# therealadityashankar/hey-buddy

Measured on AMD Instinct MI355X. Metric: audio clips/sec featurized+trained, 1.5 s @16 kHz, 1/2/4/8 GPU, higher is better.
Workload: dtype f32

## Files before the change

### hey-buddy_amd/csrc/hbk_augment_plan.h

```cpp
#pragma once

#include <algorithm>
#include <cmath>
#include <cstdarg>
#include <cstdint>
#include <cstdio>
#include <numeric>
#include <string>
#include <vector>

namespace hbk {
namespace {

constexpr int kPlanOk = 0, kPlanErrArg = -1, kPlanErrUnsupported = -3;

inline std::string strf(const char* fmt, ...) {
  char buf[512];
  va_list ap;
  va_start(ap, fmt);
  vsnprintf(buf, sizeof(buf), fmt, ap);
  va_end(ap);
  return buf;
}

// ... 79 lines not shown
    return kPlanErrUnsupported;
  }
  return kPlanOk;
}

struct PitchLayout {
  int64_t y = 0;
  int64_t taps = 0;
  int64_t yr = 0;
  int64_t sp = 0;
  int64_t key = 0;
  int64_t ord = 0;
  int64_t gord = 0;
  int64_t total = 0;
};

inline PitchLayout pitch_layout(const PitchGeometry& a, int64_t n) {
  PitchLayout w;
  w.y = 0;
  w.taps = up256(n * a.l1 * 4);
  w.yr = w.taps + up256(int64_t(kPsPhaseMax) * kPsTapMax * 4);
  w.sp = w.yr + up256(n * 8);
  w.key = w.sp + up256(n * 8);
  w.ord = w.key + up256(n * 8);
  w.gord = w.ord + up256(n * 4);
  w.total = w.gord + up256(n * 4);
  return w;
}

struct PitchKnobs {
  bool span = true;
  bool pair = true;
  bool resample_valu = false;
};

struct Grid {
  unsigned x = 1, y = 1, block = 0;
};

struct PitchLaunches {
  bool pair = false;
  int groups = 0;
  Grid taps, span, rank_clips, group, rank_groups, vocoder, resample;
  bool resample_mfma = true;
};

inline PitchLaunches pitch_launches(const PitchGeometry& a, int64_t n, const PitchKnobs& k) {
  PitchLaunches p;
  p.pair = k.span && k.pair;
  p.groups = static_cast<int>((n + kPvClips - 1) / kPvClips);
  p.taps = Grid{unsigned((a.nw * kPsTapMax + 255) / 256), 1, 256};
  p.span = Grid{unsigned((n + 3) / 4), 1, 256};
  p.rank_clips = Grid{unsigned((n + 63) / 64), 1, 1024};
  p.group = Grid{unsigned((p.groups + 255) / 256), 1, 256};
  p.rank_groups = Grid{unsigned((p.groups + 63) / 64), 1, 1024};
  p.vocoder = Grid{unsigned(p.groups), 1, unsigned(128 * kPvClips)};
  const int res_frames = (a.L + a.nw - 1) / a.nw;
  p.resample_mfma = !(k.resample_valu || a.nw > 128);
  p.resample = p.resample_mfma ? Grid{unsigned((res_frames + kRsFrames - 1) / kRsFrames), unsigned(n), 256}
                               : Grid{unsigned((res_frames + kPsResFrames - 1) / kPsResFrames), unsigned(n), 128};
  return p;
}

struct BandStopLayout {
  int64_t sums = 0;
  int64_t taps = 0;
// ... 74 lines not shown
```

### hey-buddy_amd/csrc/hbk_pitch.hip

```cpp
#include <atomic>
#include <cstdlib>

#include "hbk_augment_plan.h"
#include "hbk_common.h"

namespace hbk {
namespace {

static_assert(kPsTapMax == HBK_PITCH_SHIFT_MAX_TAPS, "the resampler's tap rows");
static_assert(kPlanOk == HBK_OK && kPlanErrArg == HBK_ERR_ARG && kPlanErrUnsupported == HBK_ERR_UNSUPPORTED,
              "the planner's status values");
#ifndef HBK_PV_ABLATE
#define HBK_PV_ABLATE 0
#endif
#ifndef HBK_PV_F32STATE
#define HBK_PV_F32STATE 0
#endif
#ifndef HBK_PV_RESTART
#if HBK_PV_F32STATE
#define HBK_PV_RESTART 128
#else
#define HBK_PV_RESTART 1024
#endif
#endif
constexpr int kPvRestart = HBK_PV_RESTART;
#if HBK_PV_F32STATE
typedef float pv_t;
#else
typedef double pv_t;
#endif

struct PitchArgs {
  const float* x;
  int64_t x_stride;
// ... 679 lines not shown
  }
  float tp[kPsTapMax];
  const float* tr = a.taps + min(ph, a.nw - 1) * kPsTapMax;
#pragma unroll
  for (int q = 0; q < kPsTapMax; ++q) tp[q] = tr[q];
  __syncthreads();
  if (ph >= a.nw) return;
  float* out = a.out + static_cast<int64_t>(a.idx[e]) * a.out_stride;
  for (int p = 0; p < kPairs; ++p) {
    const int i = (f0 + 2 * p) * a.nw + ph, i1 = i + a.nw;
    if (i >= a.L) break;
    cf v = {0.f, 0.f};
    if (i < a.target) {
      const float4* w = reinterpret_cast<const float4*>(ys2[p]);
#pragma unroll
      for (int q2 = 0; q2 < kPsTapMax / 2; ++q2) {
        const float4 ww = w[q2];
        v = __builtin_elementwise_fma(cf{tp[2 * q2], tp[2 * q2]}, cf{ww.x, ww.y}, v);
        v = __builtin_elementwise_fma(cf{tp[2 * q2 + 1], tp[2 * q2 + 1]}, cf{ww.z, ww.w}, v);
      }
    }
    out[i] = v.x;
    if (i1 < a.L) out[i1] = i1 < a.target ? v.y : 0.f;
  }
}


typedef _Float16 rs_h8 __attribute__((ext_vector_type(8)));
typedef float rs_f4 __attribute__((ext_vector_type(4)));
__device__ __forceinline__ void rs_split(float v, _Float16& h, _Float16& l) {
  h = static_cast<_Float16>(v);
  l = static_cast<_Float16>(v - static_cast<float>(h));
}
__global__ void __launch_bounds__(256) ps_resample_mfma_kernel(PitchArgs a) {
  __shared__ __attribute__((aligned(16))) _Float16 wh[kRsFrames][kRsLd];
  __shared__ __attribute__((aligned(16))) _Float16 wl[kRsFrames][kRsLd];
  __shared__ float red[4];
  const int tid = threadIdx.x, lane = tid & 63, wave = tid >> 6;
  const int e = blockIdx.y, f0 = blockIdx.x * kRsFrames;
  const float* y = a.y + static_cast<int64_t>(e) * a.l1;
  const int2 yr = a.yr[e];
  if (ps_window_silent(a, yr, e, f0 * a.orig - a.width, f0, kRsFrames, tid, 256)) return;
  constexpr int kPairs = kRsFrames * kRsK / 2, kPer = kPairs / 256;
  float v0[kPer], v1[kPer];
  float mx = 0.f;
#pragma unroll
  for (int u = 0; u < kPer; ++u) {
    const int p = tid + 256 * u, fr = p / (kRsK / 2), q = 2 * (p - fr * (kRsK / 2));
    const int src = (f0 + fr) * a.orig - a.width + q;
    const int s0 = min(max(src, 0), a.l1 - 1), s1 = min(max(src + 1, 0), a.l1 - 1);
    const float x0 = y[s0], x1 = y[s1];
    v0[u] = (src >= yr.x && src < yr.y && q < kPsTapMax) ? x0 : 0.f;
    v1[u] = (src + 1 >= yr.x && src + 1 < yr.y && q + 1 < kPsTapMax) ? x1 : 0.f;
    mx = fmaxf(mx, fmaxf(fabsf(v0[u]), fabsf(v1[u])));
  }
  const int n = lane & 15, kq = lane >> 4;
  rs_h8 bh[2][5], bl[2][5];
#pragma unroll
  for (int t = 0; t < 2; ++t) {
    const int ph = min(16 * (2 * wave + t) + n, a.nw - 1);
    const float* tr = a.taps + ph * kPsTapMax;
#pragma unroll
    for (int ks = 0; ks < 5; ++ks)
#pragma unroll
      for (int j = 0; j < 8; ++j) {
        const int q = 32 * ks + 8 * kq + j;
        const float tv = tr[min(q, kPsTapMax - 1)];
        _Float16 h, l;
        rs_split(q < kPsTapMax ? tv * 1024.f : 0.f, h, l);
        bh[t][ks][j] = h;
        bl[t][ks][j] = l;
      }
  }
  for (int o = 32; o >= 1; o >>= 1) mx = fmaxf(mx, __shfl_xor(mx, o, 64));
  if (lane == 0) red[wave] = mx;
  __syncthreads();
  mx = fmaxf(fmaxf(red[0], red[1]), fmaxf(red[2], red[3]));
  const int ex = mx > 0.f ? min(14 - ilogbf(mx), 100) : 0;
  const float scale = ldexpf(1.f, ex), unscale = ldexpf(1.f, -ex - 10);
#pragma unroll
  for (int u = 0; u < kPer; ++u) {
    const int p = tid + 256 * u, fr = p / (kRsK / 2), q = 2 * (p - fr * (kRsK / 2));
    _Float16 h0, l0, h1, l1;
    rs_split(v0[u] * scale, h0, l0);
    rs_split(v1[u] * scale, h1, l1);
    wh[fr][q] = h0;
    wh[fr][q + 1] = h1;
    wl[fr][q] = l0;
    wl[fr][q + 1] = l1;
  }
  __syncthreads();
  float* out = a.out + static_cast<int64_t>(a.idx[e]) * a.out_stride;
#pragma unroll
  for (int ft = 0; ft < kRsFrames / 16; ++ft) {
    rs_f4 acc[2] = {{0.f, 0.f, 0.f, 0.f}, {0.f, 0.f, 0.f, 0.f}};
#pragma unroll
    for (int ks = 0; ks < 5; ++ks) {
      const rs_h8 ah = *reinterpret_cast<const rs_h8*>(&wh[16 * ft + n][32 * ks + 8 * kq]);
      const rs_h8 al = *reinterpret_cast<const rs_h8*>(&wl[16 * ft + n][32 * ks + 8 * kq]);
#pragma unroll
      for (int t = 0; t < 2; ++t) {
        acc[t] = __builtin_amdgcn_mfma_f32_16x16x32_f16(ah, bh[t][ks], acc[t], 0, 0, 0);
        acc[t] = __builtin_amdgcn_mfma_f32_16x16x32_f16(ah, bl[t][ks], acc[t], 0, 0, 0);
        acc[t] = __builtin_amdgcn_mfma_f32_16x16x32_f16(al, bh[t][ks], acc[t], 0, 0, 0);
      }
    }
#pragma unroll
    for (int t = 0; t < 2; ++t) {
      const int ph = 16 * (2 * wave + t) + n;
#pragma unroll
      for (int j = 0; j < 4; ++j) {
        const int i = (f0 + 16 * ft + 4 * kq + j) * a.nw + ph;
        if (ph < a.nw && i < a.L) out[i] = i < a.target ? acc[t][j] * unscale : 0.f;
      }
    }
  }
}

PitchKnobs read_pitch_knobs() {
  PitchKnobs k;
  const char* s = getenv("HBK_PS_SPAN");
  k.span = !(s && s[0] == '0');
  s = getenv("HBK_PS_PAIR");
  k.pair = !(s && s[0] == '0');
  k.resample_valu = getenv("HBK_PS_RESAMPLE_VALU") != nullptr;
  return k;
}

int vocoder_lds_opt_in() {
  constexpr int kDevices = 64;
  static std::atomic<bool> done[kDevices];
  int dev = -1;
  HBK_HIP(hipGetDevice(&dev));
  const bool tracked = dev >= 0 && dev < kDevices;
  if (tracked && done[dev].load(std::memory_order_acquire)) return HBK_OK;
  HBK_HIP(hipFuncSetAttribute(reinterpret_cast<const void*>(ps_vocoder_kernel),
                              hipFuncAttributeMaxDynamicSharedMemorySize, int(sizeof(PvShared))));
  if (tracked) done[dev].store(true, std::memory_order_release);
  return HBK_OK;
}

template <typename... Params, typename... Args>
void launch(void (*kernel)(Params...), const Grid& g, size_t lds, hipStream_t st, Args... args) {
  hipLaunchKernelGGL(kernel, dim3(g.x, g.y), dim3(g.block), lds, st, args...);
}

}

#ifdef HBK_PHASE_TIMING
int pv_phase_take(unsigned long long* out) {
  if (hipMemcpyFromSymbol(out, HIP_SYMBOL(g_pv_phase), sizeof(unsigned long long) * 5) != hipSuccess) return -2;
  unsigned long long z[5] = {};
  (void)hipMemcpyToSymbol(HIP_SYMBOL(g_pv_phase), z, sizeof(z));
  return 0;
}
#endif

}

extern "C" {

int64_t hbk_pitch_shift_workspace_size(int64_t n, int64_t T, int32_t sample_rate, int32_t num, int32_t den) {
  hbk::PitchGeometry g;
  std::string err;
  if (n <= 0 || hbk::pitch_geometry(T, sample_rate, num, den, g, err) != HBK_OK) return 0;
  return hbk::pitch_layout(g, n).total;
}

int hbk_pitch_shift(const float* x, int64_t x_stride, int64_t n, const int32_t* idx, int64_t T, int32_t sample_rate,
                    int32_t num, int32_t den, float* out, int64_t out_stride, void* workspace,
                    int64_t workspace_bytes, void* stream) {
  using namespace hbk;
  if (n < 0) return arg_error("negative n");
  if (n == 0) return HBK_OK;
  if (n > 65535) return arg_error("n > 65535 per call");
  if (!x || !idx || !out || !workspace) return arg_error("NULL pointer");
  PitchGeometry g;
// ... 2 lines not shown
  if (rc != HBK_OK) {
    set_error("%s", err.c_str());
    return rc;
  }
  if (x_stride < T || out_stride < T) return arg_error("stride < T");
  const PitchLayout off = pitch_layout(g, n);
  if (workspace_bytes < off.total) return arg_error("workspace too small (hbk_pitch_shift_workspace_size)");
  const PitchKnobs knobs = read_pitch_knobs();
  const PitchLaunches L = pitch_launches(g, n, knobs);
  unsigned char* w = static_cast<unsigned char*>(workspace);
  PitchArgs a{};
  a.x = x;
  a.x_stride = x_stride;
  a.idx = idx;
  a.n = static_cast<int>(n);
  a.out = out;
  a.out_stride = out_stride;
  a.L = g.L, a.f_in = g.f_in, a.f_out = g.f_out, a.l1 = g.l1;
  a.orig = g.orig, a.nw = g.nw, a.width = g.width, a.target = g.target;
  a.rate = g.rate;
  a.y = reinterpret_cast<float*>(w + off.y);
  a.taps = reinterpret_cast<float*>(w + off.taps);
  a.yr = reinterpret_cast<int2*>(w + off.yr);
  a.span = knobs.span ? 1 : 0;
  if (L.pair) {
    a.sp = reinterpret_cast<int2*>(w + off.sp);
    a.key = reinterpret_cast<uint64_t*>(w + off.key);
    a.ord = reinterpret_cast<int32_t*>(w + off.ord);
    a.gord = reinterpret_cast<int32_t*>(w + off.gord);
  }
  const int lds_rc = vocoder_lds_opt_in();
  if (lds_rc != HBK_OK) return lds_rc;
  hipStream_t st = as_stream(stream);
  launch(ps_taps_kernel, L.taps, 0, st, a);
  HBK_LAUNCH_CHECK("ps_taps_kernel");
  if (L.pair) {
    launch(ps_span_kernel, L.span, 0, st, a);
    HBK_LAUNCH_CHECK("ps_span_kernel");
    launch(ps_rank_kernel, L.rank_clips, 0, st, static_cast<const uint64_t*>(a.key), a.n, a.ord);
    HBK_LAUNCH_CHECK("ps_rank_kernel");
    launch(ps_group_kernel, L.group, 0, st, a, L.groups);
    HBK_LAUNCH_CHECK("ps_group_kernel");
    launch(ps_rank_kernel, L.rank_groups, 0, st, static_cast<const uint64_t*>(a.key), L.groups, a.gord);
    HBK_LAUNCH_CHECK("ps_rank_kernel");
  }
  launch(ps_vocoder_kernel, L.vocoder, sizeof(PvShared), st, a);
  HBK_LAUNCH_CHECK("ps_vocoder_kernel");
  launch(L.resample_mfma ? ps_resample_mfma_kernel : ps_resample_kernel, L.resample, 0, st, a);
  HBK_LAUNCH_CHECK(L.resample_mfma ? "ps_resample_mfma_kernel" : "ps_resample_kernel");
  return HBK_OK;
}

}
```

### hey-buddy_amd/heybuddy/_native.py

```python
from __future__ import annotations

import ctypes
import os
import threading
from typing import Optional

import torch

__all__ = ["HBKError", "HBKUnavailable", "lib", "check", "stream_ptr", "require_device",
           "LIB_PATH"]

LIB_PATH = os.environ.get(
    "HBK_LIB",
    os.path.join(os.path.dirname(os.path.dirname(os.path.abspath(__file__))), "lib", "libhbk.so"),
)


class HBKError(RuntimeError):
    """A libhbk.so entry point returned a non-zero status."""


class HBKUnavailable(HBKError):
    """libhbk.so (or a HIP device) is not available: the HIP path cannot run."""


_lock = threading.Lock()
_lib: Optional[ctypes.CDLL] = None

_c_int64 = ctypes.c_int64
_c_int = ctypes.c_int
_c_float = ctypes.c_float
_vp = ctypes.c_void_p

_PROTOS = {
# ... 19 lines not shown
                                     ctypes.POINTER(ctypes.c_double),
                                     ctypes.POINTER(ctypes.c_double),
                                     ctypes.POINTER(ctypes.c_int32)]),
    "hbk_embed_workspace_size": (_c_int, [_vp, _c_int64, ctypes.POINTER(_c_int64)]),
    "hbk_embed_clips": (_c_int, [_vp, _vp, _c_int64, _c_int64, _vp, _vp, _c_int64, _vp]),
    "hbk_embed_split_info": (_c_int, [_vp, ctypes.c_int32, ctypes.POINTER(_c_int64)]),
    "hbk_embed_clips_front": (_c_int, [_vp, _vp, _c_int64, _c_int64, ctypes.c_int32, _vp, _vp, _c_int64, _vp]),
    "hbk_embed_clips_back": (_c_int, [_vp, _vp, _c_int64, ctypes.c_int32, _vp, _vp, _c_int64, _vp]),
    "hbk_embed_windows": (_c_int, [_vp, _vp, _c_int64, _vp, _vp, _c_int64, _vp]),
    "hbk_nan_rows_workspace_size": (_c_int64, [_c_int64]),
    "hbk_nan_rows_fix": (_c_int, [_vp, _c_int64, _c_int64, ctypes.c_uint64, _vp, _c_int64, _vp]),
    "hbk_embed_range_status": (_c_int, [_vp, ctypes.POINTER(ctypes.c_int32), ctypes.c_int32, _vp]),
    "hbk_reverb_plan_create": (_c_int, [_c_int64, ctypes.POINTER(_vp)]),
    "hbk_reverb_plan_destroy": (_c_int, [_vp]),
    "hbk_reverb_spectrum": (_c_int, [_vp, _vp, _c_int64, _c_int64, _vp, _vp]),
    "hbk_augment": (_c_int, [_vp, _vp, _c_int64, _c_int64, _vp, _c_int64, _vp, _vp, _vp, _vp, _vp,
                             _vp, _c_int64, _vp]),
    "hbk_colored_noise": (_c_int, [_vp, _vp, _c_int64, _c_int64, _vp, _c_int64, ctypes.c_uint64, _c_int64, _vp,
                                   _vp, _c_float, _vp, _c_int64, _vp, _c_int64, _vp]),
    "hbk_augment_colored": (_c_int, [_vp, _vp, _c_int64, _c_int64, _vp, _c_int64, _vp, _vp, _vp, _vp, _vp,
                                     _vp, _c_int64, ctypes.c_uint64, _c_int64, _vp, _vp, _c_float, _vp, _c_int64,
                                     _vp, _c_int64, _vp, _c_int64, _vp]),
    "hbk_colored_noise_workspace_size": (_c_int64, [_c_int64, _c_int64]),
    "hbk_colored_noise_ws": (_c_int, [_vp, _vp, _c_int64, _c_int64, _vp, _c_int64, ctypes.c_uint64, _c_int64, _vp,
                                      _vp, _c_float, _vp, _c_int64, _vp, _c_int64, _vp, _c_int64, _vp]),
    "hbk_tanh_distortion": (_c_int, [_vp, _c_int64, _c_int64, _vp, _vp, _c_int64, _vp, _c_int64, _vp]),
    "hbk_band_stop_workspace_size": (_c_int64, [_c_int64, ctypes.c_int32, ctypes.c_int32, _vp]),
    "hbk_band_stop": (_c_int, [_vp, _vp, _c_int64, _c_int64, _vp, _vp, ctypes.c_int32, _vp, _vp, _vp, _vp,
                               ctypes.c_int32, _vp, _vp, _vp, _c_int64, _vp, _c_int64, _vp]),
    "hbk_pitch_shift_workspace_size": (_c_int64, [_c_int64, _c_int64, ctypes.c_int32, ctypes.c_int32,
                                                  ctypes.c_int32]),
    "hbk_pitch_shift": (_c_int, [_vp, _c_int64, _c_int64, _vp, _c_int64, ctypes.c_int32, ctypes.c_int32,
                                 ctypes.c_int32, _vp, _c_int64, _vp, _c_int64, _vp]),
    "hbk_seven_band_eq": (_c_int, [_vp, _c_int64, _c_int64, _vp, _vp, _c_int64, _vp, _c_int64, _vp]),
    "hbk_place_clips": (_c_int, [_vp, _c_int64, _c_int64, _vp, _vp, _vp, _c_int64, _c_int64, _vp]),
    "hbk_place_clips_idx": (_c_int, [_vp, _c_int64, _c_int64, _vp, _vp, _vp, _c_int64, _vp, _c_int64, _c_int64,
                                     _vp]),
    "hbk_seven_band_eq_src": (_c_int, [_vp, _c_int64, _c_int64, _vp, _vp, _c_int64, _vp, _c_int64,
                                       _vp, _c_int64, _vp, _vp, _vp]),
    "hbk_tanh_distortion_src": (_c_int, [_vp, _c_int64, _c_int64, _vp, _vp, _c_int64, _vp, _c_int64,
                                         _vp, _c_int64, _vp, _vp, _vp]),
    "hbk_reverb_plan_set_source": (_c_int, [_vp, _vp, _c_int64, _vp, _vp]),
    "hbk_mlp_set_step_scalars": (_c_int, [_vp, _vp]),
    "hbk_mlp_plan_create": (_c_int, [ctypes.c_int32] * 4 + [ctypes.POINTER(_vp)]),
    "hbk_mlp_plan_create_ex": (_c_int, [ctypes.c_int32] * 6 + [ctypes.POINTER(_vp)]),
    "hbk_mlp_act_forward": (_c_int, [_vp, _c_int64, ctypes.c_int32, ctypes.c_int32, ctypes.c_int32, _vp, _vp]),
    "hbk_mlp_act_backward": (_c_int, [_vp, _vp, _c_int64, ctypes.c_int32, ctypes.c_int32, ctypes.c_int32, _vp,
                                      _vp]),
    "hbk_mlp_plan_create_half": (_c_int, [ctypes.c_int32] * 6 + [_vp, ctypes.POINTER(_vp)]),
    "hbk_mlp_half_layout": (_c_int, [_vp, _vp, ctypes.c_int32]),
    "hbk_mlp_plan_destroy": (_c_int, [_vp]),
    "hbk_mlp_layout": (_c_int, [_vp, ctypes.POINTER(_c_int64), _vp, ctypes.c_int32]),
    "hbk_mlp_workspace_size": (_c_int, [_vp, _c_int64, ctypes.POINTER(_c_int64)]),
    "hbk_mlp_forward": (_c_int, [_vp, _vp, _vp, _c_int64, _vp, _vp, _c_float, ctypes.c_uint64,
                                 _vp, _c_int64, _vp]),
    "hbk_mlp_train_fwd_bwd": (_c_int, [_vp, _vp, _vp, _vp, _c_int64, _c_float, _c_float, _c_float,
                                       _c_float, ctypes.c_uint64, _vp, _vp, _vp, _c_int64, _vp]),
    "hbk_mlp_gate_adam": (_c_int, [_vp, _vp, _vp, _vp, _vp, _vp, _vp, _vp, ctypes.c_int32,
                                   _c_float, _c_float, _c_float, _c_float, _vp]),
    "hbk_mlp_fused_supported": (_c_int, [_vp, ctypes.POINTER(ctypes.c_int32)]),
    "hbk_mlp_step_variant": (_c_int, [_vp, _c_int64, _vp, ctypes.POINTER(ctypes.c_int32)]),
    "hbk_mlp_step_plan_info": (_c_int, [_vp, _c_int64, _vp, ctypes.POINTER(ctypes.c_int32), ctypes.c_int32]),
    "hbk_mlp_step_fwd_bwd": (_c_int, [_vp, _vp, _vp, _c_int64, _vp, _c_int64, _vp, _c_int64, _vp, _c_int64,
                                      _c_int64, _vp, ctypes.c_int32, _vp, _c_int64, _c_float, _c_float,
                                      _c_float, _c_float, ctypes.c_uint64, _vp, _vp, _c_int64, ctypes.c_int32,
                                      _vp, _c_int64, _vp]),
# ... 14 lines not shown


class GraphOp(ctypes.Structure):
    _fields_ = [
        ("kind", ctypes.c_int32), ("kh", ctypes.c_int32), ("kw", ctypes.c_int32),
        ("cin", ctypes.c_int32), ("cout", ctypes.c_int32), ("act", ctypes.c_int32),
        ("alpha", ctypes.c_float), ("weight", _vp), ("bias", _vp),
    ]


def exported_symbols() -> list[str]:
    return list(_PROTOS)


def lib() -> ctypes.CDLL:
    global _lib
    if _lib is not None:
        return _lib
    with _lock:
        if _lib is not None:
            return _lib
        if not os.path.exists(LIB_PATH):
            raise HBKUnavailable(
                f"libhbk.so not found at {LIB_PATH}; build it with "
                "`python hey-buddy_amd/build.py` (the HIP path has no fallback)")
        try:
            handle = ctypes.CDLL(LIB_PATH, mode=ctypes.RTLD_GLOBAL)
        except OSError as e:
            raise HBKUnavailable(f"cannot load {LIB_PATH}: {e}") from e
        for name, (res, args) in _PROTOS.items():
            fn = getattr(handle, name)
            fn.restype = res
            fn.argtypes = args
        _lib = handle
        return _lib


def check(rc: int, what: str = "") -> None:
    if rc != 0:
        msg = lib().hbk_last_error().decode(errors="replace")
        raise HBKError(f"{what}: status {rc}: {msg}")


def require_device(device: Optional[torch.device | int] = None) -> torch.device:
    lib()
    if not torch.cuda.is_available():
        raise HBKUnavailable("no HIP device visible: the hey-buddy MI355X path needs a GPU")
    if device is None:
        return torch.device("cuda", torch.cuda.current_device())
    if isinstance(device, int):
        return torch.device("cuda", device)
    device = torch.device(device)
    if device.type != "cuda":
        raise HBKUnavailable(f"device {device} is not a HIP device")
    return device if device.index is not None else torch.device("cuda", torch.cuda.current_device())


def stream_ptr(device: Optional[torch.device] = None) -> int:
    return torch.cuda.current_stream(device).cuda_stream


def ptr(t: torch.Tensor) -> int:
    return t.data_ptr()
```

### include/hbk.h

```cpp
#ifndef HBK_H
#define HBK_H

#include <stdint.h>

#ifdef __cplusplus
extern "C" {
#endif

typedef enum {
  HBK_OK = 0,
  HBK_ERR_ARG = -1,
  HBK_ERR_HIP = -2,
  HBK_ERR_UNSUPPORTED = -3
} hbk_status;

const char* hbk_version(void);
const char* hbk_last_error(void);
int hbk_device_count(int* count);
int hbk_stream_create_cu_mask(const uint32_t* cu_mask, int n_words, void** stream);
int hbk_stream_destroy(void* stream);

int hbk_profile_mark(int32_t tag, void* stream);

typedef struct hbk_mel_plan hbk_mel_plan;
// ... 157 lines not shown
                const float* noise_ring, int64_t ring_len, const int64_t* noise_off,
                const float* snr_db, const float* spectra, const int32_t* spec_idx,
                const float* gain, float* out, int64_t out_stride, void* stream);

int hbk_colored_noise(const hbk_reverb_plan* plan, const float* x, int64_t n_clips, int64_t x_stride,
                      const float* white, int64_t white_stride, uint64_t seed, int64_t clips_per_noise,
                      const float* f_decay, const float* snr_db, float sample_rate, const int32_t* idx,
                      int64_t n_entries, float* out, int64_t out_stride, void* stream);
int64_t hbk_colored_noise_workspace_size(int64_t n_clips, int64_t clips_per_noise);
int hbk_colored_noise_ws(const hbk_reverb_plan* plan, const float* x, int64_t n_clips, int64_t x_stride,
                         const float* white, int64_t white_stride, uint64_t seed, int64_t clips_per_noise,
                         const float* f_decay, const float* snr_db, float sample_rate, const int32_t* idx,
                         int64_t n_entries, float* out, int64_t out_stride, void* workspace, int64_t workspace_bytes,
                         void* stream);

int hbk_augment_colored(const hbk_reverb_plan* plan, const float* x, int64_t n_clips, int64_t x_stride,
                        const float* noise_ring, int64_t ring_len, const int64_t* noise_off,
                        const float* snr_db, const float* spectra, const int32_t* spec_idx,
                        const float* gain, const float* white, int64_t white_stride, uint64_t seed,
                        int64_t clips_per_noise, const float* c_f_decay, const float* c_snr_db,
                        float sample_rate, const int32_t* c_idx, int64_t c_n_entries, float* out,
                        int64_t out_stride, void* workspace, int64_t workspace_bytes, void* stream);

#define HBK_BAND_STOP_CIRCULAR_MAX_HALF 512
#define HBK_BAND_STOP_PARTITION_TAPS 11521
int64_t hbk_band_stop_workspace_size(int64_t n, int32_t n_filters, int32_t n_spectra, void* stream);
int hbk_band_stop(const hbk_reverb_plan* plan, const float* x, int64_t x_stride, int64_t n, const int32_t* idx,
                  const int32_t* filt, int32_t n_filters, const float* f_lo, const float* f_hi,
                  const int32_t* f_half, const int32_t* f_spec0, int32_t n_spectra, const int32_t* s_filt,
                  const int32_t* s_part, float* out, int64_t out_stride, void* workspace, int64_t workspace_bytes,
                  void* stream);

#define HBK_PITCH_SHIFT_MAX_TAPS 144
int64_t hbk_pitch_shift_workspace_size(int64_t n, int64_t T, int32_t sample_rate, int32_t num, int32_t den);
int hbk_pitch_shift(const float* x, int64_t x_stride, int64_t n, const int32_t* idx, int64_t T, int32_t sample_rate,
                    int32_t num, int32_t den, float* out, int64_t out_stride, void* workspace,
                    int64_t workspace_bytes, void* stream);

int hbk_seven_band_eq(const float* x, int64_t n_clips, int64_t x_stride, const double* coef, const int32_t* idx,
                      int64_t n_entries, float* out, int64_t out_stride, void* stream);

int hbk_tanh_distortion(const float* x, int64_t n_clips, int64_t x_stride, const float* amount,
                        const int32_t* idx, int64_t n_entries, float* out, int64_t out_stride, void* stream);

int hbk_place_clips(const float* src, int64_t n_clips, int64_t src_stride, const int32_t* src_len,
                    const int32_t* pre, float* out, int64_t out_stride, int64_t T, void* stream);
int hbk_place_clips_idx(const float* src, int64_t n_clips, int64_t src_stride, const int32_t* src_len,
                        const int32_t* pre, const int32_t* idx, int64_t n_entries, float* out,
                        int64_t out_stride, int64_t T, void* stream);

int hbk_seven_band_eq_src(const float* x, int64_t n_clips, int64_t x_stride, const double* coef,
                          const int32_t* idx, int64_t n_entries, float* out, int64_t out_stride,
                          const float* src, int64_t src_stride, const int32_t* src_len,
                          const int32_t* src_pre, void* stream);
int hbk_tanh_distortion_src(const float* x, int64_t n_clips, int64_t x_stride, const float* amount,
                            const int32_t* idx, int64_t n_entries, float* out, int64_t out_stride,
                            const float* src, int64_t src_stride, const int32_t* src_len,
                            const int32_t* src_pre, void* stream);
int hbk_reverb_plan_set_source(hbk_reverb_plan* plan, const float* src, int64_t src_stride,
                               const int32_t* src_len, const int32_t* src_pre);

#ifdef __cplusplus
}
#endif

#endif
// ... 1 lines not shown
```

### hey-buddy_amd/csrc/hbk_clip_ops.hip

```cpp
#include <algorithm>

#include "hbk_aug_dev.h"

namespace hbk {
namespace {

struct TanhArgs {
  const float* x;
  int64_t x_stride;
  float* out;
  int64_t out_stride;
  int64_t n_clips;
  const float* amount;
  const int32_t* idx;
  int64_t n_entries;
  SrcView view;
};

__device__ __forceinline__ unsigned abs_bits(float v, int s) {
  return s < kT ? (__builtin_bit_cast(unsigned, v) & 0x7FFFFFFFu) : 0xFFFFFFFFu;
}

__global__ void __launch_bounds__(kThreads) __attribute__((amdgpu_waves_per_eu(8)))
tanh_distortion_kernel(TanhArgs a) {
  __shared__ unsigned hist[4096];
  __shared__ float red[32];
  __shared__ unsigned pick[2];
  constexpr int kPer = (kT + kThreads - 1) / kThreads;
  const int64_t n_iter = a.idx ? a.n_entries : a.n_clips;
  for (int64_t e = blockIdx.x; e < n_iter; e += gridDim.x) {
    const int64_t clip = a.idx ? a.idx[e] : e;
    const int tid = opaque_tid();
    const float* x = a.x + clip * a.x_stride;
    float* out = a.out + clip * a.out_stride;
    const float amt = a.amount[clip];
    if (amt != amt) {
      if (out != x) copy_clip(x, out, tid);
      continue;
    }
    float xr[kPer];
    const int pre = a.view.pre ? a.view.pre[clip] : -1, len = a.view.pre ? a.view.len[clip] : 0;
    if (pre >= 0) {
      const int n = min(len, kT);
      const float* row = n > 0 ? a.view.src + clip * a.view.stride : x;
      const int t = opaque_tid();
      const int w0 = __builtin_amdgcn_readfirstlane(t & ~63);
#pragma unroll
      for (int u = 0; u < kPer; ++u) xr[u] = load_placed_wave(row, pre, n, w0 + u * kThreads, t & 63);
    } else {
    const int t = opaque_tid();
#pragma unroll
    for (int u = 0; u < kPer; ++u) {
      const int s = t + u * kThreads;
      xr[u] = s < kT ? *reinterpret_cast<const float*>(reinterpret_cast<const char*>(x) + (static_cast<uint32_t>(s) << 2))
                     : 0.f;
    }
    }
    const double pos = (100.0 - 99.0 * static_cast<double>(amt)) / 100.0 * (kT - 1);
    const int lo = min(max(static_cast<int>(floor(pos)), 0), kT - 1);
    const double frac = pos - lo;
    unsigned prefix = 0, mask = 0, rank = static_cast<unsigned>(lo);
#pragma unroll 1
    for (int p = 0; p < 3; ++p) {
      const int shift = p == 0 ? 19 : (p == 1 ? 9 : 0), bins = p == 0 ? 4096 : (p == 1 ? 1024 : 512);
      const int per_lane = bins >> 6;
      for (int i = tid; i < bins; i += kThreads) hist[i] = 0;
      __syncthreads();
      const int t = opaque_tid();
#pragma unroll
      for (int u = 0; u < kPer; ++u) {
        const unsigned b = abs_bits(xr[u], t + u * kThreads);
        if ((b & mask) == prefix && b != 0xFFFFFFFFu) atomicAdd(&hist[(b >> shift) & (bins - 1)], 1u);
      }
      __syncthreads();
      if (tid < 64) {
        unsigned own = 0;
        for (int i = 0; i < per_lane; ++i) own += hist[per_lane * tid + i];
        unsigned inc = own;
#pragma unroll
        for (int d = 1; d < 64; d <<= 1) {
          const unsigned v = __shfl_up(inc, d, 64);
          if (tid >= d) inc += v;
        }
        const unsigned long long hit = __ballot(inc > rank);
        const int l = __ffsll(static_cast<long long>(hit)) - 1;
        if (tid == l) {
          unsigned r = rank - (inc - own), dsel = per_lane * l;
          for (int i = 0; i < per_lane - 1; ++i) {
            const unsigned h = hist[dsel];
            if (r < h) break;
            r -= h;
            ++dsel;
          }
          pick[0] = dsel;
          pick[1] = r;
        }
      }
      __syncthreads();
      prefix |= pick[0] << shift;
      mask |= static_cast<unsigned>(bins - 1) << shift;
      rank = pick[1];
    }
    float cnt = 0.f, mg = __builtin_inff();
    const int t2 = opaque_tid();
#pragma unroll
    for (int u = 0; u < kPer; ++u) {
// ... 197 lines not shown
  if (items >= (int64_t(1) << 31)) return arg_error("too many clips for one launch");
  const int64_t blocks = items;
  hipLaunchKernelGGL(place_kernel, dim3(unsigned(blocks)), dim3(256), 0, as_stream(stream), src, src_stride, src_len,
                     pre, idx, out, out_stride, n_rows, int(T));
  HBK_LAUNCH_CHECK("place_kernel");
  return HBK_OK;
}

int hbk_place_clips(const float* src, int64_t n_clips, int64_t src_stride, const int32_t* src_len,
                    const int32_t* pre, float* out, int64_t out_stride, int64_t T, void* stream) {
  return hbk_place_clips_idx(src, n_clips, src_stride, src_len, pre, nullptr, 0, out, out_stride, T, stream);
}

int hbk_tanh_distortion_src(const float* x, int64_t n_clips, int64_t x_stride, const float* amount,
                            const int32_t* idx, int64_t n_entries, float* out, int64_t out_stride,
                            const float* src, int64_t src_stride, const int32_t* src_len, const int32_t* src_pre,
                            void* stream) {
  using namespace hbk;
  if (n_clips < 0) return arg_error("negative n_clips");
  if (n_clips == 0) return HBK_OK;
  if (!x || !out || !amount) return arg_error("NULL pointer");
  if (x_stride < kT || out_stride < kT) return arg_error("stride < 23040");
  TanhArgs a;
  a.x = x;
  a.x_stride = x_stride;
  a.out = out;
  a.out_stride = out_stride;
  a.n_clips = n_clips;
  a.amount = amount;
  a.idx = idx;
  a.n_entries = idx ? n_entries : n_clips;
  const int st = src_view(src, src_stride, src_len, src_pre, a.view);
  if (st != HBK_OK) return st;
  if (a.n_entries <= 0) return n_entries < 0 ? arg_error("negative n_entries") : HBK_OK;
  const int64_t blocks = std::min<int64_t>(a.n_entries, persistent_blocks(2, stream));
  hipLaunchKernelGGL(tanh_distortion_kernel, dim3(unsigned(blocks)), dim3(kThreads), 0, as_stream(stream), a);
  HBK_LAUNCH_CHECK("tanh_distortion_kernel");
  return HBK_OK;
}

int hbk_tanh_distortion(const float* x, int64_t n_clips, int64_t x_stride, const float* amount,
                        const int32_t* idx, int64_t n_entries, float* out, int64_t out_stride, void* stream) {
  return hbk_tanh_distortion_src(x, n_clips, x_stride, amount, idx, n_entries, out, out_stride, nullptr, 0, nullptr,
                                 nullptr, stream);
}

int hbk_seven_band_eq_src(const float* x, int64_t n_clips, int64_t x_stride, const double* coef, const int32_t* idx,
                          int64_t n_entries, float* out, int64_t out_stride, const float* src, int64_t src_stride,
                          const int32_t* src_len, const int32_t* src_pre, void* stream) {
  using namespace hbk;
  if (n_clips < 0 || n_entries < 0) return arg_error("negative count");
  if (!idx) n_entries = n_clips;
  if (n_entries == 0) return HBK_OK;
  if (!x || !out || !coef) return arg_error("NULL pointer");
  if (x_stride < kT || out_stride < kT) return arg_error("stride < 23040");
  if ((reinterpret_cast<uintptr_t>(x) | reinterpret_cast<uintptr_t>(out)) % 16 || x_stride % 4 || out_stride % 4)
    return arg_error("x / out rows must be 16-B aligned");
  EqArgs a;
  a.x = x;
  a.x_stride = x_stride;
  a.coef = coef;
  a.idx = idx;
  a.out = out;
  a.out_stride = out_stride;
  a.n = n_entries;
  const int st = src_view(src, src_stride, src_len, src_pre, a.view);
// ... 15 lines not shown
```

### hey-buddy_amd/csrc/hbk_embed.hip

```cpp
#include <algorithm>
#include <cmath>
#include <cstring>
#include <numeric>
#include <vector>

#include "hbk_common.h"
#include "hbk_embed_args.h"
#include "hbk_embed_plan.h"

namespace hbk {
namespace {

constexpr int kWaves = kThreads / 64;
constexpr int kChunkClips = 16384;
inline int64_t chunk_clips() {
  static const int64_t c = [] {
    const char* e = getenv("HBK_EMBED_CHUNK");
    const long long v = e ? atoll(e) : 0;
    return v >= 256 && v <= 32768 ? int64_t(v) : int64_t(kChunkClips);
  }();
  return c;
}

typedef float f4 __attribute__((ext_vector_type(4)));
// ... 2173 lines not shown
              return &a;
            },
            args);
        const int64_t tasks = ((n_img + L.imgs_per_task - 1) / L.imgs_per_task) * L.n_bands;
        const int64_t blocks = std::min<int64_t>(tasks, persistent_blocks(s->blocks_per_cu, stream));
        if (blocks > 0) {
          (void)hipLaunchKernel(s->fn, dim3(unsigned(blocks)), dim3(L.threads), &argp, L.lds_bytes, stream);
          HBK_LAUNCH_CHECK(L.name);
        }
        break;
      }
    }
    if (prog.gather_buf >= 0 && k_end == n_ch) {
      const int n_out = static_cast<int>(prog.gather_src.size());
      const int row = static_cast<int>(out_unit_floats / n_out);
      hipLaunchKernelGGL(embed_gather_kernel, dim3(unsigned((nu + 3) / 4)), dim3(256), 0, stream,
                         bufs[prog.gather_buf], out + u0 * out_unit_floats, d_gather, nu, prog.n_src, n_out, row);
      HBK_LAUNCH_CHECK("embed_gather_kernel");
    }
  }
  return HBK_OK;
}

int run_units(const hbk_embed_plan* p, bool clips, const float* in, int64_t n, int64_t in_stride, int64_t min_stride,
              float* out, int64_t out_floats, void* workspace, int64_t workspace_bytes, void* stream, int k_begin = 0,
              int k_end = -1) {
  if (n < 0) return arg_error(clips ? "negative n_clips" : "negative n");
  if (n == 0) return HBK_OK;
  if (!in || !out || !workspace) return arg_error("NULL pointer");
  if (in_stride < min_stride) return arg_error("mel_clip_stride < seq_frames * in_w");
  int64_t need = 0;
  hbk_embed_workspace_size(p, n, &need);
  if (workspace_bytes < need) return arg_error("workspace too small");
  return run_program(clips ? p->host.clip : p->host.win, clips ? p->clip : p->win, p->d_gather, in, n, in_stride, out,
                     out_floats, static_cast<float*>(workspace), std::min<int64_t>(n, chunk_clips()),
                     as_stream(stream), p->d_range, k_begin, k_end);
}

}
}

extern "C" {

int hbk_embed_plan_create(const hbk_graph_op* ops, int32_t n_ops, int32_t in_h, int32_t in_w,
                          const int32_t* win_start, int32_t n_win, hbk_embed_plan** plan) {
  return hbk_embed_plan_create_ex(ops, n_ops, in_h, in_w, win_start, n_win, HBK_PREC_SPLIT_F16, plan);
}

int hbk_embed_plan_create_ex(const hbk_graph_op* ops, int32_t n_ops, int32_t in_h, int32_t in_w,
                             const int32_t* win_start, int32_t n_win, int32_t precision,
                             hbk_embed_plan** plan) {
  using namespace hbk;
  if (!plan) return arg_error("plan is NULL");
  *plan = nullptr;
  if (precision != HBK_PREC_SPLIT_F16 && precision != HBK_PREC_EXACT_F32) return arg_error("unknown precision");
  if (!ops || n_ops <= 0) return arg_error("empty graph");
  if (in_h <= 0 || in_w <= 0) return arg_error("bad window size");
  if (!win_start || n_win <= 0 || n_win > kMaxWin) return arg_error("n_win must be in [1, 32]");
  auto* p = new hbk_embed_plan();
  auto fail = [&](int rc) {
    hbk_embed_plan_destroy(p);
    return rc;
  };
  const EmbedKnobs knobs = read_embed_knobs();
  std::vector<OpIn> graph;
  for (int i = 0; i < n_ops; ++i) {
    const hbk_graph_op& o = ops[i];
    graph.push_back(OpIn{o.kind, o.kh, o.kw, o.cin, o.cout, o.act, o.alpha, o.weight, o.bias});
// ... 279 lines not shown
```

### hey-buddy_amd/csrc/hbk_embed_plan.h

```cpp
#pragma once

#include <algorithm>
#include <cmath>
#include <cstdarg>
#include <cstdio>
#include <cstring>
#include <initializer_list>
#include <numeric>
#include <optional>
#include <string>
#include <variant>
#include <vector>

#include "hbk_embed_args.h"

namespace hbk {
namespace {

constexpr int kPlanOk = 0, kPlanErrArg = -1, kPlanErrUnsupported = -3;
constexpr int kOpConv = 0, kOpMaxPool = 1;

struct EmbedKnobs {
  bool lds_kb_set = false;
  int lds_kb = 0;
// ... 952 lines not shown
          const int ph = int(std::find(phases.begin(), phases.end(), r % S) - phases.begin());
          const int row = (r - r % S) / S;
          ok = ok && row < t.h;
          win_src.push_back(ph * t.h + row);
        }
        p.clip.n_src = int(phases.size()) * t.h;
      }
      if (!ok) phases.clear();
    }
    const int64_t pre_floats = int64_t(pre.h) * pre.w * pre.c;
    if (!phases.empty()) {
      p.clip.gather_src = win_src;
      rc = plan_segment(ops, split, n_ops, Dims{H, wd.w, wd.c}, int(phases.size()), phases, pre_floats,
                        pre.w * pre.c, split_f16, knobs, p.clip, nullptr, err);
      p.dedup_debug = strf("hbk tail dedup: %zu phase images of %d rows per clip for %d windows\n", phases.size(), H,
                           n_win);
    } else {
      rc = plan_segment(ops, split, n_ops, Dims{wd.h, wd.w, wd.c}, n_win, roff, pre_floats, pre.w * pre.c, split_f16,
                        knobs, p.clip, nullptr, err);
    }
    if (rc) return rc;
    for (size_t k = 0; k < p.clip.chains.size(); ++k)
      (k < n_pre ? p.prefix_macs : p.tail_macs) += p.clip.chains[k].macs_per_img;
    if (!phases.empty()) p.tail_macs *= double(phases.size()) / double(n_win);
    assign_buffers(p.clip, true, n_win);
  }
  rc = plan_segment(ops, 0, n_ops, Dims{in_h, in_w, 1}, 1, {0}, int64_t(in_h) * in_w, in_w, split_f16, knobs, p.win,
                    nullptr, err);
  if (rc) return rc;
  assign_buffers(p.win, false, 1);
  return kPlanOk;
}

}
}
```

Baseline: 1.146 million.

## Cache precomputed MFMA resampler tap fragments per device and shift ratio

Result: no change. 1.148 million, median of 2 (+0.1%).

```diff
diff --git a/hey-buddy_amd/csrc/hbk_augment_plan.h b/hey-buddy_amd/csrc/hbk_augment_plan.h
--- a/hey-buddy_amd/csrc/hbk_augment_plan.h
+++ b/hey-buddy_amd/csrc/hbk_augment_plan.h
@@ -135,6 +135,7 @@
   bool span = true;
   bool pair = true;
   bool resample_valu = false;
+  bool frags = true;
 };
 
 struct Grid {
diff --git a/hey-buddy_amd/csrc/hbk_pitch.hip b/hey-buddy_amd/csrc/hbk_pitch.hip
--- a/hey-buddy_amd/csrc/hbk_pitch.hip
+++ b/hey-buddy_amd/csrc/hbk_pitch.hip
@@ -1,5 +1,7 @@
 #include <atomic>
 #include <cstdlib>
+#include <mutex>
+#include <vector>
 
 #include "hbk_augment_plan.h"
 #include "hbk_common.h"
@@ -745,7 +747,37 @@
   h = static_cast<_Float16>(v);
   l = static_cast<_Float16>(v - static_cast<float>(h));
 }
-__global__ void __launch_bounds__(256) ps_resample_mfma_kernel(PitchArgs a) {
+constexpr int kRsFragVecs = (kPsPhaseMax / 16) * (kRsK / 32) * 64;
+constexpr size_t kRsFragBytes = 2 * size_t(kRsFragVecs) * 16;
+
+__device__ __forceinline__ void rs_tap_split(const float* tr, int ks, int kq, int j, _Float16& h, _Float16& l) {
+  const int q = 32 * ks + 8 * kq + j;
+  const float tv = tr[min(q, kPsTapMax - 1)];
+  rs_split(q < kPsTapMax ? tv * 1024.f : 0.f, h, l);
+}
+
+__global__ void __launch_bounds__(256) ps_frags_kernel(const float* taps, int nw, void* frags_out) {
+  rs_h8* frags = static_cast<rs_h8*>(frags_out);
+  const int i = blockIdx.x * 256 + threadIdx.x;
+  if (i >= kRsFragVecs) return;
+  const int lane = i & 63, ks = (i >> 6) % (kRsK / 32), tl = (i >> 6) / (kRsK / 32);
+  const int n = lane & 15, kq = lane >> 4;
+  const float* tr = taps + min(16 * tl + n, nw - 1) * kPsTapMax;
+  rs_h8 h8, l8;
+#pragma unroll
+  for (int j = 0; j < 8; ++j) {
+    _Float16 h, l;
+    rs_tap_split(tr, ks, kq, j, h, l);
+    h8[j] = h;
+    l8[j] = l;
+  }
+  frags[i] = h8;
+  frags[kRsFragVecs + i] = l8;
+}
+
+template <bool kCached>
+__global__ void __launch_bounds__(256) ps_resample_mfma_kernel(PitchArgs a, const void* frags_in) {
+  const rs_h8* frags = static_cast<const rs_h8*>(frags_in);
   __shared__ __attribute__((aligned(16))) _Float16 wh[kRsFrames][kRsLd];
   __shared__ __attribute__((aligned(16))) _Float16 wl[kRsFrames][kRsLd];
   __shared__ float red[4];
@@ -757,33 +789,58 @@
   constexpr int kPairs = kRsFrames * kRsK / 2, kPer = kPairs / 256;
   float v0[kPer], v1[kPer];
   float mx = 0.f;
+  if (kCached) {
+#pragma unroll
+    for (int u = 0; u < kPer; ++u) {
+      const int p = tid + 256 * u, fr = p / (kRsK / 2), q = 2 * (p - fr * (kRsK / 2));
+      const int src = (f0 + fr) * a.orig - a.width + q;
+      v0[u] = y[min(max(src, 0), a.l1 - 1)];
+      v1[u] = y[min(max(src + 1, 0), a.l1 - 1)];
+    }
+  }
+  const int n = lane & 15, kq = lane >> 4;
+  rs_h8 bh[2][5], bl[2][5];
+#pragma unroll
+  for (int t = 0; t < 2; ++t) {
+    if (kCached) {
+#pragma unroll
+      for (int ks = 0; ks < 5; ++ks) {
+        const int v = ((2 * wave + t) * 5 + ks) * 64 + lane;
+        bh[t][ks] = frags[v];
+        bl[t][ks] = frags[kRsFragVecs + v];
+      }
+      continue;
+    }
+    const int ph = min(16 * (2 * wave + t) + n, a.nw - 1);
+    const float* tr = a.taps + ph * kPsTapMax;
+#pragma unroll
+    for (int ks = 0; ks < 5; ++ks)
+#pragma unroll
+      for (int j = 0; j < 8; ++j) {
+        _Float16 h, l;
+        rs_tap_split(tr, ks, kq, j, h, l);
+        bh[t][ks][j] = h;
+        bl[t][ks][j] = l;
+      }
+  }
+  if (kCached) {
+#pragma unroll
+    for (int u = 0; u < kPer; ++u) asm volatile("" : "+v"(v0[u]), "+v"(v1[u]));
+  }
 #pragma unroll
   for (int u = 0; u < kPer; ++u) {
     const int p = tid + 256 * u, fr = p / (kRsK / 2), q = 2 * (p - fr * (kRsK / 2));
     const int src = (f0 + fr) * a.orig - a.width + q;
-    const int s0 = min(max(src, 0), a.l1 - 1), s1 = min(max(src + 1, 0), a.l1 - 1);
-    const float x0 = y[s0], x1 = y[s1];
+    float x0, x1;
+    if (kCached) {
+      x0 = v0[u], x1 = v1[u];
+    } else {
+      const int s0 = min(max(src, 0), a.l1 - 1), s1 = min(max(src + 1, 0), a.l1 - 1);
+      x0 = y[s0], x1 = y[s1];
+    }
     v0[u] = (src >= yr.x && src < yr.y && q < kPsTapMax) ? x0 : 0.f;
     v1[u] = (src + 1 >= yr.x && src + 1 < yr.y && q + 1 < kPsTapMax) ? x1 : 0.f;
     mx = fmaxf(mx, fmaxf(fabsf(v0[u]), fabsf(v1[u])));
-  }
-  const int n = lane & 15, kq = lane >> 4;
-  rs_h8 bh[2][5], bl[2][5];
-#pragma unroll
-  for (int t = 0; t < 2; ++t) {
-    const int ph = min(16 * (2 * wave + t) + n, a.nw - 1);
-    const float* tr = a.taps + ph * kPsTapMax;
-#pragma unroll
-    for (int ks = 0; ks < 5; ++ks)
-#pragma unroll
-      for (int j = 0; j < 8; ++j) {
-        const int q = 32 * ks + 8 * kq + j;
-        const float tv = tr[min(q, kPsTapMax - 1)];
-        _Float16 h, l;
-        rs_split(q < kPsTapMax ? tv * 1024.f : 0.f, h, l);
-        bh[t][ks][j] = h;
-        bl[t][ks][j] = l;
-      }
   }
   for (int o = 32; o >= 1; o >>= 1) mx = fmaxf(mx, __shfl_xor(mx, o, 64));
   if (lane == 0) red[wave] = mx;
@@ -837,7 +894,98 @@
   s = getenv("HBK_PS_PAIR");
   k.pair = !(s && s[0] == '0');
   k.resample_valu = getenv("HBK_PS_RESAMPLE_VALU") != nullptr;
+  s = getenv("HBK_PS_FRAGS");
+  k.frags = !(s && s[0] == '0');
   return k;
+}
+
+struct RsFrags {
+  int sample_rate = 0, num = 0, den = 0;
+  rs_h8* d = nullptr;
+  hipEvent_t ready = nullptr;
+  bool done = false;
+};
+constexpr int kRsCacheDevices = 64;
+struct RsCache {
+  std::mutex mu;
+  std::vector<RsFrags> e[kRsCacheDevices];
+};
+RsCache& rs_cache() {
+  static RsCache* c = new RsCache;
+  return *c;
+}
+
+template <typename... Params, typename... Args>
+void launch(void (*kernel)(Params...), const Grid& g, size_t lds, hipStream_t st, Args... args) {
+  hipLaunchKernelGGL(kernel, dim3(g.x, g.y), dim3(g.block), lds, st, args...);
+}
+
+int rs_frags_get(const PitchArgs& a, const Grid& taps_grid, int sample_rate, int num, int den, hipStream_t st,
+                 const rs_h8** frags) {
+  *frags = nullptr;
+  int dev = -1;
+  HBK_HIP(hipGetDevice(&dev));
+  if (dev < 0 || dev >= kRsCacheDevices) return HBK_OK;
+  RsCache& c = rs_cache();
+  std::lock_guard<std::mutex> lock(c.mu);
+  for (RsFrags& f : c.e[dev]) {
+    if (f.sample_rate != sample_rate || f.num != num || f.den != den) continue;
+    if (!f.done) {
+      const hipError_t q = hipEventQuery(f.ready);
+      if (q == hipSuccess) {
+        f.done = true;
+      } else if (q == hipErrorNotReady) {
+        HBK_HIP(hipStreamWaitEvent(st, f.ready, 0));
+      } else {
+        return hip_error(q, "hipEventQuery(resampler fragments)");
+      }
+    }
+    *frags = f.d;
+    return HBK_OK;
+  }
+  RsFrags f;
+  f.sample_rate = sample_rate, f.num = num, f.den = den;
+  HBK_HIP(hipMalloc(reinterpret_cast<void**>(&f.d), kRsFragBytes));
+  hipError_t e = hipEventCreateWithFlags(&f.ready, hipEventDisableTiming);
+  if (e == hipSuccess) {
+    launch(ps_taps_kernel, taps_grid, 0, st, a);
+    launch(ps_frags_kernel, Grid{unsigned((kRsFragVecs + 255) / 256), 1, 256}, 0, st,
+           static_cast<const float*>(a.taps), a.nw, static_cast<void*>(f.d));
+    e = hipGetLastError();
+    if (e == hipSuccess) e = hipEventRecord(f.ready, st);
+  }
+  if (e != hipSuccess) {
+    if (f.ready) (void)hipEventDestroy(f.ready);
+    (void)hipFree(f.d);
+    return hip_error(e, "resampler fragments");
+  }
+  c.e[dev].push_back(f);
+  *frags = f.d;
+  return HBK_OK;
+}
+
+int rs_cache_clear() {
+  RsCache& c = rs_cache();
+  std::lock_guard<std::mutex> lock(c.mu);
+  int cur = -1;
+  bool moved = false;
+  int rc = HBK_OK;
+  for (int dev = 0; dev < kRsCacheDevices; ++dev) {
+    if (c.e[dev].empty()) continue;
+    if (cur < 0) HBK_HIP(hipGetDevice(&cur));
+    hipError_t e = hipSuccess;
+    if (dev != cur || moved) e = hipSetDevice(dev), moved = true;
+    if (e == hipSuccess) e = hipDeviceSynchronize();
+    for (RsFrags& f : c.e[dev]) {
+      (void)hipEventDestroy(f.ready);
+      const hipError_t fe = hipFree(f.d);
+      if (e == hipSuccess) e = fe;
+    }
+    c.e[dev].clear();
+    if (e != hipSuccess && rc == HBK_OK) rc = hip_error(e, "hbk_pitch_cache_clear");
+  }
+  if (moved) (void)hipSetDevice(cur);
+  return rc;
 }
 
 int vocoder_lds_opt_in() {
@@ -851,11 +999,6 @@
                               hipFuncAttributeMaxDynamicSharedMemorySize, int(sizeof(PvShared))));
   if (tracked) done[dev].store(true, std::memory_order_release);
   return HBK_OK;
-}
-
-template <typename... Params, typename... Args>
-void launch(void (*kernel)(Params...), const Grid& g, size_t lds, hipStream_t st, Args... args) {
-  hipLaunchKernelGGL(kernel, dim3(g.x, g.y), dim3(g.block), lds, st, args...);
 }
 
 }
@@ -924,8 +1067,15 @@
   const int lds_rc = vocoder_lds_opt_in();
   if (lds_rc != HBK_OK) return lds_rc;
   hipStream_t st = as_stream(stream);
-  launch(ps_taps_kernel, L.taps, 0, st, a);
-  HBK_LAUNCH_CHECK("ps_taps_kernel");
+  const rs_h8* frags = nullptr;
+  if (L.resample_mfma && knobs.frags) {
+    const int frc = rs_frags_get(a, L.taps, sample_rate, num, den, st, &frags);
+    if (frc != HBK_OK) return frc;
+  }
+  if (!frags) {
+    launch(ps_taps_kernel, L.taps, 0, st, a);
+    HBK_LAUNCH_CHECK("ps_taps_kernel");
+  }
   if (L.pair) {
     launch(ps_span_kernel, L.span, 0, st, a);
     HBK_LAUNCH_CHECK("ps_span_kernel");
@@ -938,9 +1088,16 @@
   }
   launch(ps_vocoder_kernel, L.vocoder, sizeof(PvShared), st, a);
   HBK_LAUNCH_CHECK("ps_vocoder_kernel");
-  launch(L.resample_mfma ? ps_resample_mfma_kernel : ps_resample_kernel, L.resample, 0, st, a);
+  if (!L.resample_mfma)
+    launch(ps_resample_kernel, L.resample, 0, st, a);
+  else if (frags)
+    launch(ps_resample_mfma_kernel<true>, L.resample, 0, st, a, static_cast<const void*>(frags));
+  else
+    launch(ps_resample_mfma_kernel<false>, L.resample, 0, st, a, static_cast<const void*>(frags));
   HBK_LAUNCH_CHECK(L.resample_mfma ? "ps_resample_mfma_kernel" : "ps_resample_kernel");
   return HBK_OK;
 }
 
-}
+int hbk_pitch_cache_clear(void) { return hbk::rs_cache_clear(); }
+
+}
diff --git a/hey-buddy_amd/heybuddy/_native.py b/hey-buddy_amd/heybuddy/_native.py
--- a/hey-buddy_amd/heybuddy/_native.py
+++ b/hey-buddy_amd/heybuddy/_native.py
@@ -1,5 +1,6 @@
 from __future__ import annotations
 
+import atexit
 import ctypes
 import os
 import threading
@@ -85,6 +86,7 @@
                                                   ctypes.c_int32]),
     "hbk_pitch_shift": (_c_int, [_vp, _c_int64, _c_int64, _vp, _c_int64, ctypes.c_int32, ctypes.c_int32,
                                  ctypes.c_int32, _vp, _c_int64, _vp, _c_int64, _vp]),
+    "hbk_pitch_cache_clear": (_c_int, []),
     "hbk_seven_band_eq": (_c_int, [_vp, _c_int64, _c_int64, _vp, _vp, _c_int64, _vp, _c_int64, _vp]),
     "hbk_place_clips": (_c_int, [_vp, _c_int64, _c_int64, _vp, _vp, _vp, _c_int64, _c_int64, _vp]),
     "hbk_place_clips_idx": (_c_int, [_vp, _c_int64, _c_int64, _vp, _vp, _vp, _c_int64, _vp, _c_int64, _c_int64,
@@ -165,6 +167,7 @@
             fn = getattr(handle, name)
             fn.restype = res
             fn.argtypes = args
+        atexit.register(handle.hbk_pitch_cache_clear)
         _lib = handle
         return _lib
 
diff --git a/include/hbk.h b/include/hbk.h
--- a/include/hbk.h
+++ b/include/hbk.h
@@ -213,6 +213,7 @@
                   void* stream);
 
 #define HBK_PITCH_SHIFT_MAX_TAPS 144
+int hbk_pitch_cache_clear(void);
 int64_t hbk_pitch_shift_workspace_size(int64_t n, int64_t T, int32_t sample_rate, int32_t num, int32_t den);
 int hbk_pitch_shift(const float* x, int64_t x_stride, int64_t n, const int32_t* idx, int64_t T, int32_t sample_rate,
                     int32_t num, int32_t den, float* out, int64_t out_stride, void* workspace,
```

## Pick embed chunk size to minimize idle wave passes; aggregate zero-bin histogram atomics

Applied to the files above, without the earlier changes.

Result: faster. 1.138 million before, 1.150 million after, median of 6 (+1.1%).

```diff
diff --git a/hey-buddy_amd/csrc/hbk_clip_ops.hip b/hey-buddy_amd/csrc/hbk_clip_ops.hip
--- a/hey-buddy_amd/csrc/hbk_clip_ops.hip
+++ b/hey-buddy_amd/csrc/hbk_clip_ops.hip
@@ -1,4 +1,5 @@
 #include <algorithm>
+#include <cstdlib>
 
 #include "hbk_aug_dev.h"
 
@@ -15,6 +16,7 @@
   const int32_t* idx;
   int64_t n_entries;
   SrcView view;
+  int zero_agg;
 };
 
 __device__ __forceinline__ unsigned abs_bits(float v, int s) {
@@ -67,11 +69,16 @@
       for (int i = tid; i < bins; i += kThreads) hist[i] = 0;
       __syncthreads();
       const int t = opaque_tid();
+      int zeros = 0;
 #pragma unroll
       for (int u = 0; u < kPer; ++u) {
         const unsigned b = abs_bits(xr[u], t + u * kThreads);
-        if ((b & mask) == prefix && b != 0xFFFFFFFFu) atomicAdd(&hist[(b >> shift) & (bins - 1)], 1u);
-      }
+        const bool match = (b & mask) == prefix && b != 0xFFFFFFFFu;
+        const bool zero = match && b == 0u && a.zero_agg;
+        zeros += __popcll(__ballot(zero));
+        if (match && !zero) atomicAdd(&hist[(b >> shift) & (bins - 1)], 1u);
+      }
+      if (zeros && (t & 63) == 0) atomicAdd(&hist[0], static_cast<unsigned>(zeros));
       __syncthreads();
       if (tid < 64) {
         unsigned own = 0;
@@ -335,6 +342,8 @@
   a.n_entries = idx ? n_entries : n_clips;
   const int st = src_view(src, src_stride, src_len, src_pre, a.view);
   if (st != HBK_OK) return st;
+  const char* agg = getenv("HBK_TANH_ZERO_AGG");
+  a.zero_agg = !(agg && atoi(agg) == 0);
   if (a.n_entries <= 0) return n_entries < 0 ? arg_error("negative n_entries") : HBK_OK;
   const int64_t blocks = std::min<int64_t>(a.n_entries, persistent_blocks(2, stream));
   hipLaunchKernelGGL(tanh_distortion_kernel, dim3(unsigned(blocks)), dim3(kThreads), 0, as_stream(stream), a);
diff --git a/hey-buddy_amd/csrc/hbk_embed.hip b/hey-buddy_amd/csrc/hbk_embed.hip
--- a/hey-buddy_amd/csrc/hbk_embed.hip
+++ b/hey-buddy_amd/csrc/hbk_embed.hip
@@ -2229,8 +2229,22 @@
   int64_t need = 0;
   hbk_embed_workspace_size(p, n, &need);
   if (workspace_bytes < need) return arg_error("workspace too small");
-  return run_program(clips ? p->host.clip : p->host.win, clips ? p->clip : p->win, p->d_gather, in, n, in_stride, out,
-                     out_floats, static_cast<float*>(workspace), std::min<int64_t>(n, chunk_clips()),
+  const ProgramPlan& prog = clips ? p->host.clip : p->host.win;
+  const std::vector<ChainPlan>& dev = clips ? p->clip : p->win;
+  int64_t chunk = std::min<int64_t>(n, chunk_clips());
+  const char* round = getenv("HBK_EMBED_CHUNK_ROUND");
+  if (n > chunk && !(round && atoi(round) == 0)) {
+    const int n_ch = static_cast<int>(prog.chains.size());
+    std::vector<ChunkChain> chains;
+    for (int k = k_begin; k < (k_end < 0 ? n_ch : k_end); ++k) {
+      const Slot& s = dev[k].pattern.fn ? dev[k].pattern : dev[k].base;
+      chains.push_back(ChunkChain{persistent_blocks(s.blocks_per_cu, stream), prog.chains[k].imgs_per_unit,
+                                  s.plan->imgs_per_task, s.plan->n_bands,
+                                  prog.chains[k].macs_per_img * double(prog.chains[k].imgs_per_unit)});
+    }
+    chunk = plan_chunk(chains, n, chunk).chunk;
+  }
+  return run_program(prog, dev, p->d_gather, in, n, in_stride, out, out_floats, static_cast<float*>(workspace), chunk,
                      as_stream(stream), p->d_range, k_begin, k_end);
 }
 
diff --git a/hey-buddy_amd/csrc/hbk_embed_plan.h b/hey-buddy_amd/csrc/hbk_embed_plan.h
--- a/hey-buddy_amd/csrc/hbk_embed_plan.h
+++ b/hey-buddy_amd/csrc/hbk_embed_plan.h
@@ -1008,5 +1008,67 @@
   return kPlanOk;
 }
 
-}
-}
+struct ChunkChain {
+  int64_t blocks;
+  int64_t imgs_per_unit;
+  int imgs_per_task, n_bands;
+  double macs;
+};
+
+struct ChunkChoice {
+  int64_t chunk = 0;
+  int64_t n_full = 0;
+  int64_t last = 0;
+};
+
+inline int64_t chunk_passes(const ChunkChain& c, int64_t nu) {
+  if (nu <= 0) return 0;
+  const int64_t tasks = ((nu * c.imgs_per_unit + c.imgs_per_task - 1) / c.imgs_per_task) * c.n_bands;
+  return (tasks + c.blocks - 1) / c.blocks;
+}
+
+inline double chunk_pass_clips(const ChunkChain& c) {
+  return double(c.blocks) * c.imgs_per_task / (double(c.n_bands) * double(c.imgs_per_unit));
+}
+
+inline double chunk_idle(const std::vector<ChunkChain>& chains, int64_t n, int64_t chunk) {
+  const int64_t n_full = n / chunk, last = n - n_full * chunk;
+  double idle = 0;
+  for (const ChunkChain& c : chains) {
+    const double passes = double(n_full) * double(chunk_passes(c, chunk)) + double(chunk_passes(c, last));
+    idle += c.macs * (passes * chunk_pass_clips(c) - double(n));
+  }
+  return idle;
+}
+
+constexpr int kChunkMaxPasses = 64;
+inline ChunkChoice plan_chunk(const std::vector<ChunkChain>& chains, int64_t n, int64_t cap) {
+  ChunkChoice r;
+  cap = std::max<int64_t>(cap, 1);
+  if (n <= 0) return r;
+  int64_t best = std::min(n, cap);
+  if (n > cap) {
+    double best_idle = chunk_idle(chains, n, cap);
+    for (const ChunkChain& c : chains) {
+      if (c.blocks <= 0 || c.imgs_per_task <= 0 || c.n_bands <= 0 || c.imgs_per_unit <= 0) continue;
+      if (chunk_passes(c, cap) > kChunkMaxPasses) continue;
+      for (int64_t m = 1; m <= kChunkMaxPasses; ++m) {
+        const int64_t cand = ((m * c.blocks) / c.n_bands) * c.imgs_per_task / c.imgs_per_unit;
+        if (cand > cap) break;
+        if (cand < (cap + 1) / 2) continue;
+        const double idle = chunk_idle(chains, n, cand);
+        if (idle < best_idle || (idle == best_idle && cand > best)) {
+          best_idle = idle;
+          best = cand;
+        }
+      }
+    }
+  }
+  r.chunk = best;
+  r.n_full = n / best;
+  r.last = n - r.n_full * best;
+  return r;
+}
+
+}
+}
```
